# zhipeng-wei/Image-to-Video-I2V-attack

Hardware: AMD Instinct MI355X
Metric: adversarial frames/sec (10-step I2V, ResNet-50 layer3, 32x224^2 clips) (higher is better)
Workload: dtype f32

## Files before the change

image-to-video-i2v-attack_amd/csrc/i2v_conv_scpair.hip:

```cpp
#include "i2v_conv_tile.h"

#ifndef I2V_SCPAIR_WPE
#define I2V_SCPAIR_WPE I2V_PREF_WPE
#endif

template <int MODE_A>
__global__ void __launch_bounds__(256) __attribute__((amdgpu_waves_per_eu(I2V_SCPAIR_WPE, I2V_SCPAIR_WPE)))
conv_igemm_scpair(const I2VConvParams a, const I2VConvParams b, const int n_cd_tiles) {
    constexpr int BD = 64, BP = 64, WD = 2, WP = 2, FR = 32;
    constexpr bool PREF_A = MODE_A == 1;
    constexpr int LA = conv_lds_floats<BD, BP, WD, false, conv_deep(MODE_A, PREF_A) ? I2V_DEEP_STAGES : 2>();
    constexpr int LB = conv_lds_floats<BD, BP, WD, false, conv_deep(1, true) ? I2V_DEEP_STAGES : 2>();
    __shared__ __attribute__((aligned(16))) float smem[LA > LB ? LA : LB];
    I2V_PROBE_T probe;
    probe.entry();
    const int lid = conv_xcd_lid(blockIdx.x, gridDim.x);
    const int cd0 = (lid % n_cd_tiles) * BD;
    const int64_t px0 = (int64_t)(lid / n_cd_tiles) * BP;

    constexpr int C4 = BP / 4, RSTEP = 1024 / BP, NQ = WD * FR / RSTEP;
    float4 y[NQ];
    {
        f32x16 acc[1][1];
        float4 pre_a[PREF_A ? NQ : 1]; unsigned gw_a[PREF_A ? NQ : 1];
        conv_tile_loop<BD, BP, WD, WP, MODE_A, PREF_A>(a, cd0, px0, gridDim.x, smem, probe, blockIdx.x, I2V_PRIO_LEVELS, acc, pre_a, gw_a);
        float (*Cs)[BP] = reinterpret_cast<float (*)[BP]>(smem);
        conv_acc_to_rows<BP, WP, false>(acc[0], Cs);
        const int t = threadIdx.x, c4 = t % C4, rbase = t / C4;
        const bool pok = px0 + (int64_t)c4 * 4 < (int64_t)a.N * a.Hg * a.Wg;
#pragma unroll
        for (int q = 0; q < NQ; ++q) {
            const int row = rbase + q * RSTEP, cd = cd0 + row;
            float4 v = make_float4(0.f, 0.f, 0.f, 0.f);
            if (pok && cd < a.Cd) {
                v = *reinterpret_cast<const float4*>(&Cs[row][c4 * 4]);
                if (a.shift) { const float sh = a.shift[cd]; v.x += sh; v.y += sh; v.z += sh; v.w += sh; }
            }
            y[q] = v;
        }
        __syncthreads();
    }
    f32x16 acc[1][1];
    float4 pre0[NQ]; unsigned pregw[NQ];
    conv_tile_loop<BD, BP, WD, WP, 1, true>(b, cd0, px0, gridDim.x, smem, probe, blockIdx.x, I2V_PRIO_LEVELS, acc, pre0, pregw);
#pragma unroll
    for (int q = 0; q < NQ; ++q) pre0[q] = y[q];
    conv_vec_epilogue<BD, BP, WD, WP, true, false, false>(b, acc, cd0, px0, smem, pre0, pregw, nullptr);
    probe.exit(blockIdx.x);
}

long long g_stat_scpair = 0;

int k_conv_scpair_ok(const I2VConvParams& a, const I2VConvParams& b) { return i2v_conv_scpair_ok(a, b) ? 1 : 0; }

int k_conv_scpair(const I2VConvParams& a_in, const I2VConvParams& b_in, i2v_stream_t s) {
    I2VConvParams a = a_in, b = b_in;
    if (!i2v_conv_scpair_ok(a, b)) { snprintf(g_be_err, sizeof g_be_err, "shortcut-pair launch: the two launches do not form a pair"); g_be_has_err = true; return 1; }
    const int64_t P = (int64_t)b.N * b.Hg * b.Wg;
    if (P + 1024 >= (1ll << 31)) { snprintf(g_be_err, sizeof g_be_err, "conv launch of more than 2^31 grid pixels"); g_be_has_err = true; return 1; }
    conv_magics(a); conv_magics(b);
    b.add0 = nullptr; b.add0_nstride = 0;
    const int n_cd = (b.Cd + 63) / 64;
    const int64_t grid = (P + 63) / 64 * n_cd;
    if (grid <= 0) return 0;
    if (grid > 0x7fffffff) { snprintf(g_be_err, sizeof g_be_err, "conv grid too large"); g_be_has_err = true; return 1; }
    __atomic_fetch_add(&g_stat_scpair, 1, __ATOMIC_RELAXED);
    if (a.pointwise) hipLaunchKernelGGL((conv_igemm_scpair<1>), dim3((unsigned)grid), dim3(256), 0, (hipStream_t)s, a, b, n_cd);
    else hipLaunchKernelGGL((conv_igemm_scpair<2>), dim3((unsigned)grid), dim3(256), 0, (hipStream_t)s, a, b, n_cd);
    LAUNCH_CHECK("conv_scpair");
    return 0;
}
```

image-to-video-i2v-attack_amd/csrc/i2v_conv_tile.h:

```cpp
#pragma once
#include "i2v_be.h"

#ifndef I2V_PROBE_T
struct I2VNoProbe {
    __device__ __forceinline__ void entry() {}
    __device__ __forceinline__ void loop_begin() {}
    __device__ __forceinline__ void loop_end(int ) {}
    __device__ __forceinline__ void exit(int ) {}
};
#define I2V_PROBE_T I2VNoProbe
#endif

#ifndef I2V_PRIO_LEVELS
#define I2V_PRIO_LEVELS 3
#endif
#ifndef I2V_DEEP
#define I2V_DEEP 1
#endif
#ifndef I2V_DEEP_STAGES
#define I2V_DEEP_STAGES 3
#endif
#ifndef I2V_BF3_STAGES
#define I2V_BF3_STAGES 2
#endif
#ifndef I2V_SMALL_WPE
#define I2V_SMALL_WPE 7
#endif
#ifndef I2V_PREF_WPE
#define I2V_PREF_WPE 6
#endif
#ifndef I2V_MID_WPE
#define I2V_MID_WPE 5
#endif
#ifndef I2V_TALL_WPE
#define I2V_TALL_WPE 6
#endif
#ifndef I2V_BIG_WPE
#define I2V_BIG_WPE 3
#endif

static constexpr int conv_waves_per_simd(int BD, int BP, bool PREF, bool hi, int MODE = 0) {
    return (BD == 64 && BP == 64) ? (PREF ? (I2V_DEEP && MODE == 1 && I2V_DEEP_STAGES > 3 ? 4  : I2V_PREF_WPE) : I2V_SMALL_WPE) : (BD == 128 && BP == 64) ? I2V_TALL_WPE : (BD == 32 && BP == 256) ? 4  : BD * BP == 8192 ? I2V_MID_WPE : BD * BP == 16384 ? I2V_BIG_WPE : (hi ? 8 : 1);
}
#define I2V_CONV_WPE __attribute__((amdgpu_waves_per_eu(conv_waves_per_simd(BD, BP, PREF, false, MODE), conv_waves_per_simd(BD, BP, PREF, true, MODE))))
static constexpr bool conv_deep(int MODE, bool PREF) { return I2V_DEEP && PREF && MODE == 1; }
template <int BD, int BP, int WD, bool MF16, int NST = 2, int CPB = 1, int BF3 = 0>
constexpr int conv_lds_floats() {
    constexpr int stage = NST * CPB * (I2V_KC * BP + (BF3 == 2 ? 0 : BF3 ? ((BD / 32) * 3 + 3) / 4 * 4 * 256 : I2V_KC * BD)), epi = WD * (MF16 ? 16 : 32) * BP;
    return stage > epi ? stage : epi;
}

template <int HWM>
constexpr int conv_halo_lds_floats() {
    constexpr int stage = 2 * I2V_KC * (64 + 64 + 2 * HWM + 2), epi = 64 * 64;
    return stage > epi ? stage : epi;
}

template <int BD, int BP, int WD, bool PREF, bool MF16, bool FUSE, typename PT>
__device__ __forceinline__ void conv_vec_rows(const PT& p, const int i, const int cd0, const int64_t px0, const float (*const Cs)[BP], const int t,
                                              const float4* const pre0, const unsigned* const pregw, float* const mid) {
    constexpr int FR = MF16 ? 16 : 32;
    const int lane = t & 63;
    const int HWg = p.Hg * p.Wg, HoWo = p.Ho * p.Wo;
    const int64_t P = (int64_t)p.N * HWg;
    (void)pre0; (void)pregw; (void)mid;
#ifdef I2V_NT_ALL
    const bool nt_store = true;
#else
    const bool nt_store = p.cfg > 0 && ((p.cfg - 1) & 128);
#endif
    constexpr int C4 = BP / 4, RSTEP = 1024 / BP, NQ = WD * FR / RSTEP;
    const int c4 = t % C4, rbase = t / C4;
    const int64_t pp = px0 + (int64_t)c4 * 4;
    const bool pok = pp < P;
    const int64_t n = pok ? fastdiv((unsigned)pp, p.dv_hw_m, p.dv_hw_s) : 0;
    const int64_t poff = pp - n * HWg;
    #pragma unroll
    for (int q = 0; q < NQ; ++q) {
        const int row = rbase + q * RSTEP;
        const int cd = cd0 + (row / FR) * (BD / WD) + i * FR + (row % FR);
        const bool valid = pok && cd < p.Cd;
        float4 v = make_float4(0.f, 0.f, 0.f, 0.f);
        if (valid) {
        v = *reinterpret_cast<const float4*>(&Cs[row][c4 * 4]);
        const int64_t o = (int64_t)cd * HoWo + poff;
        if (p.gate_scale) {
            const float4 m = *reinterpret_cast<const float4*>(p.mask + n * p.mask_nstride + o);
            const float gs = p.gate_scale[cd], gt = p.gate_shift[cd];
            if (!(fmaf(m.x, gs, gt) > 0.f)) v.x = 0.f;
            if (!(fmaf(m.y, gs, gt) > 0.f)) v.y = 0.f;
            if (!(fmaf(m.z, gs, gt) > 0.f)) v.z = 0.f;
            if (!(fmaf(m.w, gs, gt) > 0.f)) v.w = 0.f;
        }
        if (p.shift) { const float sh = p.shift[cd]; v.x += sh; v.y += sh; v.z += sh; v.w += sh; }
        if (PREF) {
            v.x += pre0[q].x; v.y += pre0[q].y; v.z += pre0[q].z; v.w += pre0[q].w;
        } else {
            if (p.add0 && p.add0_stride == 1) {
                const float4 a = *reinterpret_cast<const float4*>(p.add0 + n * p.add0_nstride + o);
                v.x += a.x; v.y += a.y; v.z += a.z; v.w += a.w;
            } else if (p.add0) {
                const int oh = (int)fastdiv((unsigned)poff, p.dv_wo_m, p.dv_wo_s), ow = (int)(poff - (int64_t)oh * p.Wo);
                if (!(oh & 1) && (oh >> 1) < p.add0_H) {
                    const float2 a = *reinterpret_cast<const float2*>(
                        p.add0 + n * p.add0_nstride + (int64_t)cd * p.add0_H * p.add0_W + (oh >> 1) * p.add0_W + (ow >> 1));
                    v.x += a.x; v.z += a.y;
                }
            }
        }
        if (p.add1) {
            const float4 a = *reinterpret_cast<const float4*>(p.add1 + n * p.add1_nstride + o);
            v.x += a.x; v.y += a.y; v.z += a.z; v.w += a.w;
        }
        if (p.relu) { v.x = fmaxf(v.x, 0.f); v.y = fmaxf(v.y, 0.f); v.z = fmaxf(v.z, 0.f); v.w = fmaxf(v.w, 0.f); }
        if (p.gate) {
            const unsigned w = PREF ? pregw[q] : p.gate[(int64_t)cd * p.gate_stride + ((p.gate_pix0 + pp) >> 5)];
            const unsigned g = w >> ((unsigned)(p.gate_pix0 + pp) & 31u);
            if (!(g & 1u)) v.x = 0.f;
            if (!(g & 2u)) v.y = 0.f;
            if (!(g & 4u)) v.z = 0.f;
            if (!(g & 8u)) v.w = 0.f;
        } else if (p.mask && !p.gate_scale) {
            const float4 m = *reinterpret_cast<const float4*>(p.mask + n * p.mask_nstride + o);
            if (!(m.x > 0.f)) v.x = 0.f;
            if (!(m.y > 0.f)) v.y = 0.f;
            if (!(m.z > 0.f)) v.z = 0.f;
            if (!(m.w > 0.f)) v.w = 0.f;
        }
        if constexpr (!FUSE) {
            if (nt_store) { typedef float nt4 __attribute__((ext_vector_type(4))); const nt4 w4 = {v.x, v.y, v.z, v.w};
                            __builtin_nontemporal_store(w4, reinterpret_cast<nt4*>(p.dst + n * p.dst_nstride + o)); }
            else *reinterpret_cast<float4*>(p.dst + n * p.dst_nstride + o) = v;
        }
        }
        if constexpr (FUSE)
            *reinterpret_cast<float4*>(mid + (cd - cd0) * BP + c4 * 4) = v;
        if (p.gate_out) {
            unsigned nib = valid ? ((v.x > 0.f ? 1u : 0u) | (v.y > 0.f ? 2u : 0u) | (v.z > 0.f ? 4u : 0u) | (v.w > 0.f ? 8u : 0u)) : 0u;
            nib <<= 4 * (lane & 7);
            nib |= (unsigned)__builtin_amdgcn_update_dpp(0, (int)nib, 0xB1, 0xF, 0xF, true);
            nib |= (unsigned)__builtin_amdgcn_update_dpp(0, (int)nib, 0x4E, 0xF, 0xF, true);
            nib |= (unsigned)__builtin_amdgcn_update_dpp(0, (int)nib, 0x141, 0xF, 0xF, true);
            if (valid && (lane & 7) == 0)
                p.gate_out[(int64_t)cd * p.gate_out_stride + ((p.gate_out_pix0 + pp) >> 5)] = nib;
        }
    }
}

#define I2V_FROW(r) (MF16 ? 4 * lk + (r) : ((r) & 3) + 8 * ((r) >> 2) + 4 * lk)
template <int BP, int WP, bool MF16, int TP, typename ACC>
__device__ __forceinline__ void conv_acc_to_rows(ACC (&acc)[TP], float (*const Cs)[BP]) {
    constexpr int FR = MF16 ? 16 : 32, NR = MF16 ? 4 : 16;
    const int lane = threadIdx.x & 63, wave = threadIdx.x >> 6;
    const int wd = wave / WP, wpx = wave % WP;
    const int l31 = MF16 ? (lane & 15) : (lane & 31), lk = MF16 ? (lane >> 4) : (lane >> 5);
    __syncthreads();
#pragma unroll
    for (int j = 0; j < TP; ++j)
#pragma unroll
        for (int r = 0; r < NR; ++r)
            Cs[wd * FR + I2V_FROW(r)][wpx * (BP / WP) + j * FR + l31] = acc[j][r];
    __syncthreads();
}
template <int BD, int BP, int WD, int WP, bool PREF, bool MF16, bool FUSE, typename ACC, typename PT>
__device__ __forceinline__ void conv_vec_epilogue(const PT& p, ACC (&acc)[BD / WD / (MF16 ? 16 : 32)][BP / WP / (MF16 ? 16 : 32)], const int cd0,
                                                  const int64_t px0, float* const smem, const float4* const pre0, const unsigned* const pregw,
                                                  float* const mid) {
    constexpr int FR = MF16 ? 16 : 32, TD = BD / WD / FR;
    const int t = threadIdx.x;
    float (*Cs)[BP] = reinterpret_cast<float (*)[BP]>(smem);
#pragma unroll
    for (int i = 0; i < TD; ++i) {
        conv_acc_to_rows<BP, WP, MF16>(acc[i], Cs);
        conv_vec_rows<BD, BP, WD, PREF, MF16, FUSE>(p, i, cd0, px0, Cs, t, pre0, pregw, mid);
    }
}
#undef I2V_FROW

__device__ __forceinline__ int conv_xcd_lid(const int bid, const int nwg) {
    const int q8 = nwg >> 3, r8 = nwg & 7, xcd = bid & 7;
    return (xcd < r8 ? xcd * (q8 + 1) : r8 * (q8 + 1) + (xcd - r8) * q8) + (bid >> 3);
}

template <int BD, int BP, int WD, int WP, int MODE, bool PREF, bool PRE = false, bool VID = false, bool MF16 = false, int HWM = 0, int CPB = 1, int FUSE = 0, int BF3 = 0>
__device__ __forceinline__ void conv_tile_loop(const I2VConvParams& p, const int cd0, const int64_t px0, const int nwg, float* const smem, I2V_PROBE_T& probe,
                                               const int probe_slot, const int prio_arg,
                                               typename std::conditional<MF16, f32x4, f32x16>::type (&acc)[BD / WD / (MF16 ? 16 : 32)][BP / WP / (MF16 ? 16 : 32)],
                                               float4 (&pre0)[PREF ? WD * (MF16 ? 16 : 32) / (1024 / BP) : 1], unsigned (&pregw)[PREF ? WD * (MF16 ? 16 : 32) / (1024 / BP) : 1]) {
#if defined(__HIP_DEVICE_COMPILE__)
    constexpr int KC = I2V_KC;
    constexpr int FR = MF16 ? 16 : 32;
    constexpr int NR = MF16 ? 4 : 16;
    constexpr int TD = BD / WD / FR, TP = BP / WP / FR;
    static_assert(!(MF16 && (PRE || PREF)), "no pre-activation / prefetch variants of the 16x16 tile");
    constexpr bool DEEP = conv_deep(MODE, PREF) || (BF3 == 1 && I2V_BF3_STAGES > 2) || BF3 == 3;
    constexpr int NST = BF3 == 3 ? 3 : BF3 == 1 ? I2V_BF3_STAGES : DEEP ? I2V_DEEP_STAGES : 2, AHEAD = NST - 1;
    constexpr bool HALO = MODE == 5;
    constexpr int HS = HALO ? BP + 2 * HWM + 2 : 1, HQ = (HS + 63) / 64;
    static_assert(!HALO || (HWM > 0 && BD == 64 && BP == 64 && !PREF && !PRE && !VID && !MF16), "halo staging: the plain 64x64 image tile only");
    static_assert(CPB == 1 || (!HALO && !DEEP && !PREF && !PRE && MODE != 4 && MODE != 0), "several chunks per barrier: the plain pointwise / tap-uniform loops only");
    constexpr int KB = CPB * KC;
    static_assert(!BF3 || (!MF16 && !PRE && !PREF && !HALO && (MODE == 1 || MODE == 2) && FUSE == 0 && BD % 32 == 0), "split-bf16 K loop: the plain pointwise / tap-uniform tiles");
    constexpr int AF = BF3 == 2 ? 0 : BF3 ? CPB * (((BD / 32) * 3 + 3) / 4 * 4) * 256 : KB * BD;
    float (*As)[KB][BD] = reinterpret_cast<float (*)[KB][BD]>(smem);
    float* const As3 = smem;
    float (*Bs)[KB][BP] = reinterpret_cast<float (*)[KB][BP]>(smem + NST * AF);

    const int t = threadIdx.x, lane = t & 63, wave = t >> 6;
    const int wd = wave / WP, wpx = wave % WP;

    const int HWg = p.Hg * p.Wg;
    const int64_t P = (int64_t)p.N * HWg;

    constexpr bool PW = MODE == 1;
    constexpr bool QUAD = MODE == 4;
    typedef __attribute__((address_space(3))) void* lds_ptr_t;
    constexpr unsigned OOB = 0x80000000u;
    const int wv = __builtin_amdgcn_readfirstlane(wave);
    const __amdgpu_buffer_rsrc_t rs_w = BF3 ? __builtin_amdgcn_make_buffer_rsrc((void*)p.wp3, 0, (p.Kpad / KC) * (p.Cdpad / 32) * 3072, 0x00020000)
                                            : __builtin_amdgcn_make_buffer_rsrc((void*)p.wp, 0, p.Kpad * p.Cdpad * 4, 0x00020000);
    constexpr unsigned XB = QUAD ? 64u : 0u;
    const __amdgpu_buffer_rsrc_t rs_x = __builtin_amdgcn_make_buffer_rsrc((void*)((const char*)p.src - XB), 0, p.src_span_bytes + 2 * XB, 0x00020000);
    constexpr int NA = BF3 == 2 ? 0 : BF3 ? (BD / 32) * 3 : KC * BD / 256, NAQ = (NA + 3) / 4;
    constexpr int BPER = (PW || QUAD) ? 256 : 64;
    constexpr int NB = HALO ? 0 : KC * BP / BPER, NBQ = (NB + 3) / 4;
    const int bcol = PW ? (lane * 4) % BP : (BP >= 64 ? ((wave * 64) % BP) + lane : lane % BP);
    const int64_t ppix = px0 + bcol;
    const bool pvalid = ppix < P;
    const int64_t pn = pvalid ? fastdiv((unsigned)ppix, p.dv_hw_m, p.dv_hw_s) : 0;
    const int prem = (int)(ppix - pn * HWg);
    const int HWs = p.Hs * p.Ws;
    int h0 = 0, w0 = 0, t0 = 0;
    int64_t pns = pn;
    if (VID) {
        const int64_t clip = fastdiv((unsigned)pn, p.dv_t_m, p.dv_t_s);
        t0 = (int)(pn - clip * p.Tg) * p.st;
        pns = clip * p.Ts + t0;
    }
    const int nstr = (int)p.src_nstride;
    unsigned xoff;
    if (PW) xoff = (unsigned)((pns * p.src_nstride + prem) * 4);
    else {
        const int gi = (int)fastdiv((unsigned)prem, p.dv_w_m, p.dv_w_s), gj = prem - gi * p.Wg;
        h0 = gi * p.sh; w0 = gj * p.sw;
        xoff = (unsigned)((pns * p.src_nstride + (int64_t)h0 * p.Ws + w0) * 4) + XB;
    }
    if (!pvalid) xoff = OOB;
    unsigned aoff[NAQ ? NAQ : 1];
#pragma unroll
    for (int q = 0; q < NAQ; ++q) {
        const int f = (wave + 4 * q) * 256 + lane * 4;
        aoff[q] = BF3 ? (unsigned)(((cd0 / 32) * 3 + wave + 4 * q) * 1024 + lane * 16) : (unsigned)(((f / BD) * p.Cdpad + f % BD + cd0) * 4);
    }
    unsigned boff[PW ? NBQ : 1];
    if (PW) {
#pragma unroll
        for (int q = 0; q < NBQ; ++q) boff[q] = pvalid ? xoff + (unsigned)((((wave + 4 * q) * 256 + lane * 4) / BP) * HWs * 4) : OOB;
    }

#define I2V_ISSUE_PIECE(j_, k0_, buf_, vb_) I2V_ISSUE_PIECE_SUB(j_, k0_, buf_, vb_, 0)
#define I2V_ISSUE_PIECE_SUB(j_, k0_, buf_, vb_, sub_)                                                     \
    {                                                                                                     \
        constexpr int jj = (j_);                                                                          \
        const int k0 = (k0_);                                                                             \
        if constexpr (jj < NAQ) {                                                                         \
            const int ins = wv + 4 * jj;                                                                  \
            if constexpr (BF3) {    \
                __builtin_amdgcn_raw_ptr_buffer_load_lds(rs_w, (lds_ptr_t)(As3 + (buf_) * AF + (sub_) * (AF / CPB) + ins * 256), 16, ins < NA ? aoff[jj] : OOB, \
                                                         (k0 / KC) * (p.Cdpad / 32) * 3072, 0, 0);       \
            } else if (NA % 4 == 0 || ins < NA) {                                                         \
                if constexpr (false)                                                                      \
                    ;                                                                                     \
                else                                                                                      \
                    __builtin_amdgcn_raw_ptr_buffer_load_lds(rs_w, (lds_ptr_t)(&As[buf_][(sub_) * KC][0] + ins * 256), 16, aoff[jj],  \
                                                             k0 * p.Cdpad * 4, 0, 0);                     \
            }                                                                                             \
        } else {                                                                                          \
            constexpr int q = jj - NAQ;                                                                   \
            const int ins = wv + 4 * q;                                                                   \
            float* const bbuf = &Bs[buf_][(sub_) * KC][0];                                                \
            if (NB % 4 == 0 || ins < NB) {                                                                \
                if constexpr (PW) {                                                                       \
                    unsigned v = boff[q];                                                                 \
                    if (k0 + KC > p.K)             \
                        v = (k0 + ((wave + 4 * q) * 256 + lane * 4) / BP < p.K) ? v : OOB;                \
                    __builtin_amdgcn_raw_ptr_buffer_load_lds(rs_x, (lds_ptr_t)(bbuf + ins * 256), 16, v,         \
                                                             k0 * HWs * 4, 0, 0);                         \
                } else if constexpr (QUAD) {                                                              \
                     \
                    const I2VKEntry e = load_kentry(p.ktab, k0 + 4 * ((ins * 64) / BP));                  \
                    const int hs = h0 + e.dh, dtk = VID ? (e.valid >> 1) : 0;                             \
                    const bool ok = pvalid && (unsigned)hs < (unsigned)p.Hs && (!VID || (unsigned)(t0 + dtk) < (unsigned)p.Ts); \
                    const unsigned v = ok ? xoff + (unsigned)((e.chan_off + dtk * nstr + e.dh * p.Ws + e.dw) * 4) : OOB; \
                    __builtin_amdgcn_raw_ptr_buffer_load_lds(rs_x, (lds_ptr_t)(bbuf + ins * 256), 16, v, 0, 0, 0); \
                } else if constexpr (MODE == 2) {                                                         \
                    __builtin_amdgcn_raw_ptr_buffer_load_lds(rs_x, (lds_ptr_t)(bbuf + ins * 64), 4, vb_,         \
                                                             ((ins * 64) / BP) * HWs * 4, 0, 0);          \
                } else {                                                                                  \
                    const I2VKEntry e = load_kentry(p.ktab, k0 + (ins * 64) / BP);                        \
                    const int hs = h0 + e.dh, ws = w0 + e.dw, dtk = VID ? (e.valid >> 1) : 0;             \
                    const bool ok = pvalid && (e.valid & 1) && (unsigned)hs < (unsigned)p.Hs &&           \
                                    (unsigned)ws < (unsigned)p.Ws && (!VID || (unsigned)(t0 + dtk) < (unsigned)p.Ts); \
                    const unsigned v = ok ? xoff + (unsigned)((e.chan_off + dtk * nstr + e.dh * p.Ws + e.dw) * 4) : OOB; \
                    __builtin_amdgcn_raw_ptr_buffer_load_lds(rs_x, (lds_ptr_t)(bbuf + ins * 64), 4, v, 0, 0, 0); \
                }                                                                                         \
            }                                                                                             \
        }                                                                                                 \
    }
#define I2V_CHUNK_VB(e_)                                                                                  \
    ([&]() -> unsigned {                                                                                  \
        const int hs = h0 + (e_).dh, ws = w0 + (e_).dw, dtk = VID ? ((e_).valid >> 1) : 0;                \
        const bool ok = pvalid && (unsigned)hs < (unsigned)p.Hs && (unsigned)ws < (unsigned)p.Ws &&       \
                        (!VID || (unsigned)(t0 + dtk) < (unsigned)p.Ts);                                  \
        return ok ? xoff + (unsigned)(((e_).chan_off + dtk * nstr + (e_).dh * p.Ws + (e_).dw) * 4) : OOB; \
    }())

    constexpr int E_C4 = BP / 4, E_RSTEP = 1024 / BP, E_NQ = WD * FR / E_RSTEP;
    static_assert(!PREF || TD == 1, "PREF needs a single epilogue pass");
    static_assert(!PREF || E_NQ == WD * (MF16 ? 16 : 32) / (1024 / BP), "pre0 / pregw (the caller's): one entry per row a lane owns");
    if (PREF) {
        const int e_c4 = t % E_C4, e_rbase = t / E_C4;
        const int64_t e_pp = px0 + (int64_t)e_c4 * 4;
        const bool e_ok = e_pp < P;
        const int64_t e_n = e_ok ? fastdiv((unsigned)e_pp, p.dv_hw_m, p.dv_hw_s) : 0;
        const int64_t e_poff = e_pp - e_n * HWg;
        const int e_HoWo = p.Ho * p.Wo;
#pragma unroll
        for (int q = 0; q < E_NQ; ++q) {
            const int row = e_rbase + q * E_RSTEP;
            const int cd = cd0 + (row >> 5) * (BD / WD) + (row & 31);
            const bool ok = e_ok && cd < p.Cd;
            const int64_t o = (int64_t)cd * e_HoWo + e_poff;
            pre0[q] = (ok && p.add0) ? *reinterpret_cast<const float4*>(p.add0 + e_n * p.add0_nstride + o) : make_float4(0.f, 0.f, 0.f, 0.f);
            pregw[q] = (ok && p.gate) ? p.gate[(int64_t)cd * p.gate_stride + ((p.gate_pix0 + e_pp) >> 5)] : 0xffffffffu;
        }
    }

    probe.loop_begin();
    typedef short bf8 __attribute__((ext_vector_type(8)));
    typedef float f4 __attribute__((ext_vector_type(4)));
    constexpr int TD_ = BD / WD / (MF16 ? 16 : 32);
    bf8 wcur[BF3 == 2 ? CPB : 1][BF3 == 2 ? TD_ : 1][3];
    const char* const w3lane = BF3 ? (const char*)p.wp3 + (size_t)lane * 16 + (size_t)(cd0 / 32 + (wave / WP) * TD_) * 3072 : nullptr;
    const size_t w3chunk = BF3 ? (size_t)(p.Cdpad / 32) * 3072 : 0;
    auto load_w3 = [&](const int chunk, const int i, const int pl) {
        return __builtin_bit_cast(bf8, *reinterpret_cast<const f4*>(w3lane + (size_t)chunk * w3chunk + (i * 3 + pl) * 1024));
    };
    if constexpr (BF3 == 2) {
#pragma unroll
        for (int sb = 0; sb < CPB; ++sb)
#pragma unroll
            for (int i = 0; i < TD_; ++i)
#pragma unroll
                for (int pl = 0; pl < 3; ++pl) wcur[sb][i][pl] = load_w3(sb, i, pl);
    }
    (void)wcur; (void)w3lane; (void)w3chunk;
    constexpr int TP_ = BP / WP / (MF16 ? 16 : 32);
    bf8 xcur[BF3 == 3 ? TP_ : 1][3];
    (void)xcur;
    auto bf3_split2 = [](const float lo, const float hi, unsigned& p1, unsigned& p2, unsigned& p3) {
        typedef __bf16 bf2 __attribute__((ext_vector_type(2)));
        typedef float f2 __attribute__((ext_vector_type(2)));
        const unsigned a = __builtin_bit_cast(unsigned, __builtin_convertvector((f2){lo, hi}, bf2));
        const float rl = lo - __builtin_bit_cast(float, a << 16), rh = hi - __builtin_bit_cast(float, a & 0xffff0000u);
        const unsigned b = __builtin_bit_cast(unsigned, __builtin_convertvector((f2){rl, rh}, bf2));
        const float sl = rl - __builtin_bit_cast(float, b << 16), sh = rh - __builtin_bit_cast(float, b & 0xffff0000u);
        const unsigned c = __builtin_bit_cast(unsigned, __builtin_convertvector((f2){sl, sh}, bf2));
        p1 = a; p2 = b; p3 = c;
    };
    auto bf3_split_frag = [&](const float (&x)[8], bf8 (&out)[3]) {
        typedef unsigned u4 __attribute__((ext_vector_type(4)));
        unsigned q1[4], q2[4], q3[4];
#pragma unroll
        for (int e = 0; e < 4; ++e) bf3_split2(x[2 * e], x[2 * e + 1], q1[e], q2[e], q3[e]);
        out[0] = __builtin_bit_cast(bf8, (u4){q1[0], q1[1], q1[2], q1[3]});
        out[1] = __builtin_bit_cast(bf8, (u4){q2[0], q2[1], q2[2], q2[3]});
        out[2] = __builtin_bit_cast(bf8, (u4){q3[0], q3[1], q3[2], q3[3]});
    };
    (void)bf3_split_frag;
#pragma unroll
    for (int a = 0; a < TD; ++a)
#pragma unroll
        for (int b = 0; b < TP; ++b)
#pragma unroll
            for (int r = 0; r < NR; ++r) acc[a][b][r] = 0.f;

    const int nchunks = p.Kpad / KC;
    const int l31 = MF16 ? (lane & 15) : (lane & 31), lk = MF16 ? (lane >> 4) : (lane >> 5);
    constexpr int NL = NAQ + NBQ;
    constexpr int KR = MF16 ? 4 : 2;
    constexpr int KS = KC / KR;
    constexpr int PPS = (NL + KS - 1) / KS;
    I2VKEntry e_next[CPB];
#pragma unroll
    for (int h = 0; h < CPB; ++h) e_next[h] = I2VKEntry{0, 0, 0, 0};
    const int nsuper = nchunks / CPB;
    bool qok[QUAD ? TP : 1][2][MF16 ? 1 : 2];
    if constexpr (QUAD) {
#pragma unroll
        for (int j = 0; j < TP; ++j) {
            const int64_t fp = px0 + wpx * (BP / WP) + j * FR + l31;
            const unsigned fr = fp < P ? (unsigned)fp - fastdiv((unsigned)fp, p.dv_hw_m, p.dv_hw_s) * (unsigned)HWg : 0u;
            const int fj = (int)(fr - fastdiv(fr, p.dv_w_m, p.dv_w_s) * (unsigned)p.Wg);
#pragma unroll
            for (int qi = 0; qi < 2; ++qi)
#pragma unroll
                for (int hf = 0; hf < (MF16 ? 1 : 2); ++hf) {
                    const int el = MF16 ? lk : 2 * hf + lk;
                    qok[j][qi][hf] = 4 * qi + el < p.quad_kw && (unsigned)(fj * p.sw + p.quad_dw0 + 4 * qi + el) < (unsigned)p.Ws;
                }
        }
    }
    if constexpr (HALO) {
        constexpr int NT = 9, HPW = 4 * HQ, PPC = (HPW + NT - 1) / NT;
        float* const Hb = smem + NST * KC * BD;
        const int W_ = HWM;
        int tsh[NT], tdh[NT], tdw[NT];
#pragma unroll
        for (int t = 0; t < NT; ++t) {
            const I2VKEntry e = load_kentry(p.ktab, t * KC);
            tdh[t] = e.dh; tdw[t] = e.dw; tsh[t] = e.dh * W_ + e.dw + W_ + 1;
        }
        const int chan0 = load_kentry(p.ktab, 0).chan_off;
        const int ngroups = nchunks / NT;
        const int gstride = ngroups > 1 ? load_kentry(p.ktab, NT * KC).chan_off - chan0 : 0;
        const int64_t fp = px0 + wpx * (BP / WP) + l31;
        const bool fpv = fp < P;
        const unsigned fr = fpv ? (unsigned)fp - fastdiv((unsigned)fp, p.dv_hw_m, p.dv_hw_s) * (unsigned)HWg : 0u;
        const int fh = (int)fastdiv(fr, p.dv_w_m, p.dv_w_s), fw = (int)fr - fh * p.Wg;
        unsigned tmask = 0;
#pragma unroll
        for (int t = 0; t < NT; ++t)
            tmask |= (fpv && (unsigned)(fh + tdh[t]) < (unsigned)p.Hs && (unsigned)(fw + tdw[t]) < (unsigned)p.Ws) ? (1u << t) : 0u;
        const int lbase = lk * HS + wpx * (BP / WP) + l31;
        unsigned hoff[HQ];
#pragma unroll
        for (int q = 0; q < HQ; ++q) {
            const int64_t vp = px0 - (W_ + 1) + 64 * q + lane;
            const bool ok = vp >= 0 && vp < P;
            const int64_t vn = ok ? fastdiv((unsigned)vp, p.dv_hw_m, p.dv_hw_s) : 0;
            hoff[q] = ok ? (unsigned)((vn * p.src_nstride + (vp - vn * HWg)) * 4) : OOB;
        }
        auto halo_piece = [&]<int IDX>(std::integral_constant<int, IDX>, const int gb, const int chan_off) {
            constexpr int chl = IDX / HQ, q = IDX % HQ;
            float* const dst = Hb + ((gb * KC + wv * 4 + chl) * HS + 64 * q);
            const int so = (chan_off + (wv * 4 + chl) * HWs) * 4;
            if constexpr (chl == 3 && q == HQ - 1) {
                if (lane < HS - 64 * q) __builtin_amdgcn_raw_ptr_buffer_load_lds(rs_x, (lds_ptr_t)dst, 4, hoff[q], so, 0, 0);
            } else
                __builtin_amdgcn_raw_ptr_buffer_load_lds(rs_x, (lds_ptr_t)dst, 4, hoff[q], so, 0, 0);
        };
        if (ngroups > 0) {
            [&]<int... I>(std::integer_sequence<int, I...>) { ((halo_piece(std::integral_constant<int, I>{}, 0, chan0)), ...); }
            (std::make_integer_sequence<int, HPW>{});
            I2V_ISSUE_PIECE(0, 0, 0, OOB);
        }
        int gbuf = 0;
        for (int g = 0; g < ngroups; ++g) {
            const bool more_g = g + 1 < ngroups;
            const int chan_next = chan0 + (g + 1) * gstride;
            [&]<int... T>(std::integer_sequence<int, T...>) {
                (([&] {
                    constexpr int t = T;
                    const int abuf = (g + t) & 1;
                    asm volatile("s_waitcnt vmcnt(0)" ::: "memory");
                    asm volatile("s_waitcnt lgkmcnt(0)" ::: "memory");
                    __builtin_amdgcn_s_barrier();
                    const int hidx = lbase + gbuf * KC * HS + tsh[t];
                    const bool ok = (tmask >> t) & 1u;
                    float fa[2], fb[2];
                    auto rd = [&](const int s_, const int set) {
                        fa[set] = As[abuf][KR * s_ + lk][wd * (BD / WD) + l31];
                        fb[set] = Hb[hidx + KR * s_ * HS];
                    };
                    rd(0, 0);
                    [&]<int... S>(std::integer_sequence<int, S...>) {
                        (([&] {
                            constexpr int s_ = S, set = S & 1;
// ... 449 lines not shown
```

Measured before the change: 757.6.

## Split conv epilogue into load/math/store passes with early operand prefetch

Restructures the conv vector epilogue into separate operand-load, math and store phases, batched over row groups, so that global loads (shift, mask, residual, gate words) are issued before the accumulator-to-LDS barrier and overlap with it. The LDS staging barriers are replaced with explicit lgkmcnt waits plus raw s_barrier, which avoids waiting on outstanding global loads. The shortcut-pair kernel likewise prefetches shift values before the LDS transpose. The change adds register pressure from held operands and a configurable batching plan, while the 128x64 tile keeps the old chained path.

```diff
diff --git a/image-to-video-i2v-attack_amd/csrc/i2v_conv_scpair.hip b/image-to-video-i2v-attack_amd/csrc/i2v_conv_scpair.hip
--- a/image-to-video-i2v-attack_amd/csrc/i2v_conv_scpair.hip
+++ b/image-to-video-i2v-attack_amd/csrc/i2v_conv_scpair.hip
@@ -25,16 +25,21 @@
         float4 pre_a[PREF_A ? NQ : 1]; unsigned gw_a[PREF_A ? NQ : 1];
         conv_tile_loop<BD, BP, WD, WP, MODE_A, PREF_A>(a, cd0, px0, gridDim.x, smem, probe, blockIdx.x, I2V_PRIO_LEVELS, acc, pre_a, gw_a);
         float (*Cs)[BP] = reinterpret_cast<float (*)[BP]>(smem);
-        conv_acc_to_rows<BP, WP, false>(acc[0], Cs);
         const int t = threadIdx.x, c4 = t % C4, rbase = t / C4;
         const bool pok = px0 + (int64_t)c4 * 4 < (int64_t)a.N * a.Hg * a.Wg;
+        float sh[NQ];
+        if (a.shift) {
+#pragma unroll
+            for (int q = 0; q < NQ; ++q) { const int cd = cd0 + rbase + q * RSTEP; sh[q] = a.shift[cd < a.Cd ? cd : 0]; }
+        }
+        conv_acc_to_rows<BP, WP, false>(acc[0], Cs, t);
 #pragma unroll
         for (int q = 0; q < NQ; ++q) {
             const int row = rbase + q * RSTEP, cd = cd0 + row;
             float4 v = make_float4(0.f, 0.f, 0.f, 0.f);
             if (pok && cd < a.Cd) {
                 v = *reinterpret_cast<const float4*>(&Cs[row][c4 * 4]);
-                if (a.shift) { const float sh = a.shift[cd]; v.x += sh; v.y += sh; v.z += sh; v.w += sh; }
+                if (a.shift) { v.x += sh[q]; v.y += sh[q]; v.z += sh[q]; v.w += sh[q]; }
             }
             y[q] = v;
         }
diff --git a/image-to-video-i2v-attack_amd/csrc/i2v_conv_tile.h b/image-to-video-i2v-attack_amd/csrc/i2v_conv_tile.h
--- a/image-to-video-i2v-attack_amd/csrc/i2v_conv_tile.h
+++ b/image-to-video-i2v-attack_amd/csrc/i2v_conv_tile.h
@@ -56,8 +56,180 @@
     return stage > epi ? stage : epi;
 }
 
+struct ConvRowOps { float4 m, a0, a1; float gs, gt; unsigned gw; };
+template <int BP>
+struct ConvRowLane {
+    int c4, rbase;
+    int64_t pp, n, poff;
+    bool pok;
+    template <typename PT>
+    __device__ __forceinline__ ConvRowLane(const PT& p, const int64_t px0, const int t) {
+        c4 = t % (BP / 4); rbase = t / (BP / 4);
+        pp = px0 + (int64_t)c4 * 4;
+        pok = pp < (int64_t)p.N * (p.Hg * p.Wg);
+        n = pok ? fastdiv((unsigned)pp, p.dv_hw_m, p.dv_hw_s) : 0;
+        poff = pp - n * (p.Hg * p.Wg);
+    }
+};
+template <int BD, int BP, int WD, bool PREF, bool MF16, bool LITE, int NB, typename PT>
+__device__ __forceinline__ void conv_vec_rows_load(const PT& p, const int i, const int q0, const int cd0, const ConvRowLane<BP>& L, ConvRowOps (&ops)[NB],
+                                                   float (&sh)[WD * (MF16 ? 16 : 32) / (1024 / BP)]) {
+    constexpr int FR = MF16 ? 16 : 32, RSTEP = 1024 / BP, NQ = WD * FR / RSTEP;
+    const int HoWo = p.Ho * p.Wo;
+    int cdc[NB]; int64_t o[NB]; bool vld[NB];
+#pragma unroll
+    for (int q = 0; q < NB; ++q) {
+        const int row = L.rbase + (q0 + q) * RSTEP;
+        const int cd = cd0 + (row / FR) * (BD / WD) + i * FR + (row % FR);
+        const bool valid = L.pok && cd < p.Cd;
+        vld[q] = valid; cdc[q] = valid ? cd : 0;
+        o[q] = valid ? (int64_t)cd * HoWo + L.poff : 0;
+    }
+    if (!LITE && p.gate_scale) {
+#pragma unroll
+        for (int q = 0; q < NB; ++q) {
+            ops[q].m = *reinterpret_cast<const float4*>(p.mask + L.n * p.mask_nstride + o[q]);
+            ops[q].gs = p.gate_scale[(unsigned)cdc[q]]; ops[q].gt = p.gate_shift[(unsigned)cdc[q]];
+        }
+    }
+    if (LITE ? q0 == 0 && p.shift : p.shift != nullptr) {
+#pragma unroll
+        for (int q = LITE ? 0 : q0; q < (LITE ? NQ : q0 + NB); ++q) {
+            const int row = L.rbase + q * RSTEP;
+            const int cd = cd0 + (row / FR) * (BD / WD) + i * FR + (row % FR);
+            sh[q] = p.shift[cd < p.Cd ? (unsigned)cd : 0u];
+        }
+    }
+    if constexpr (!PREF) {
+        if (p.add0 && p.add0_stride == 1) {
+#pragma unroll
+            for (int q = 0; q < NB; ++q) ops[q].a0 = *reinterpret_cast<const float4*>(p.add0 + L.n * p.add0_nstride + o[q]);
+        } else if (p.add0) {
+            const int oh = (int)fastdiv((unsigned)L.poff, p.dv_wo_m, p.dv_wo_s), ow = (int)(L.poff - (int64_t)oh * p.Wo);
+            const bool even = !(oh & 1) && (oh >> 1) < p.add0_H;
+#pragma unroll
+            for (int q = 0; q < NB; ++q) {
+                const int64_t oc = (vld[q] && even)
+                                       ? L.n * p.add0_nstride + (int64_t)cdc[q] * p.add0_H * p.add0_W + (oh >> 1) * p.add0_W + (ow >> 1) : 0;
+                const float2 a = *reinterpret_cast<const float2*>(p.add0 + oc);
+                ops[q].a0.x = a.x; ops[q].a0.y = a.y;
+            }
+        }
+    }
+    if (p.add1) {
+#pragma unroll
+        for (int q = 0; q < NB; ++q) ops[q].a1 = *reinterpret_cast<const float4*>(p.add1 + L.n * p.add1_nstride + o[q]);
+    }
+    if (p.gate) {
+        if constexpr (!PREF) {
+            const int64_t gp = (int64_t)p.gate_pix0 + (L.pok ? L.pp : 0);
+#pragma unroll
+            for (int q = 0; q < NB; ++q) ops[q].gw = p.gate[(int64_t)cdc[q] * p.gate_stride + (gp >> 5)];
+        }
+    } else if (!LITE && p.mask && !p.gate_scale) {
+#pragma unroll
+        for (int q = 0; q < NB; ++q) ops[q].m = *reinterpret_cast<const float4*>(p.mask + L.n * p.mask_nstride + o[q]);
+    }
+}
+template <int BD, int BP, int WD, bool PREF, bool MF16, bool LITE, int NB, typename PT>
+__device__ __forceinline__ void conv_vec_rows_math(const PT& p, const int i, const int q0, const int cd0, const ConvRowLane<BP>& L, const float (*const Cs)[BP],
+                                                   const ConvRowOps (&ops)[NB], const float (&sh)[WD * (MF16 ? 16 : 32) / (1024 / BP)], const float4* const pre0,
+                                                   const unsigned* const pregw, float4 (&vv)[NB]) {
+    constexpr int FR = MF16 ? 16 : 32, RSTEP = 1024 / BP;
+    (void)pre0; (void)pregw;
+#pragma unroll
+    for (int q = 0; q < NB; ++q) {
+        const int row = L.rbase + (q0 + q) * RSTEP;
+        const int cd = cd0 + (row / FR) * (BD / WD) + i * FR + (row % FR);
+        const bool valid = L.pok && cd < p.Cd;
+        float4 v = make_float4(0.f, 0.f, 0.f, 0.f);
+        if (valid) {
+        v = *reinterpret_cast<const float4*>(&Cs[row][L.c4 * 4]);
+        if (!LITE && p.gate_scale) {
+            const float4 m = ops[q].m;
+            const float gs = ops[q].gs, gt = ops[q].gt;
+            if (!(fmaf(m.x, gs, gt) > 0.f)) v.x = 0.f;
+            if (!(fmaf(m.y, gs, gt) > 0.f)) v.y = 0.f;
+            if (!(fmaf(m.z, gs, gt) > 0.f)) v.z = 0.f;
+            if (!(fmaf(m.w, gs, gt) > 0.f)) v.w = 0.f;
+        }
+        if (p.shift) { const float s = sh[q0 + q]; v.x += s; v.y += s; v.z += s; v.w += s; }
+        if (PREF) {
+            v.x += pre0[q0 + q].x; v.y += pre0[q0 + q].y; v.z += pre0[q0 + q].z; v.w += pre0[q0 + q].w;
+        } else {
+            if (p.add0 && p.add0_stride == 1) {
+                const float4 a = ops[q].a0;
+                v.x += a.x; v.y += a.y; v.z += a.z; v.w += a.w;
+            } else if (p.add0) {
+                const int oh = (int)fastdiv((unsigned)L.poff, p.dv_wo_m, p.dv_wo_s);
+                if (!(oh & 1) && (oh >> 1) < p.add0_H) { v.x += ops[q].a0.x; v.z += ops[q].a0.y; }
+            }
+        }
+        if (p.add1) {
+            const float4 a = ops[q].a1;
+            v.x += a.x; v.y += a.y; v.z += a.z; v.w += a.w;
+        }
+        if (p.relu) { v.x = fmaxf(v.x, 0.f); v.y = fmaxf(v.y, 0.f); v.z = fmaxf(v.z, 0.f); v.w = fmaxf(v.w, 0.f); }
+        if (p.gate) {
+            const unsigned w = PREF ? pregw[q0 + q] : ops[q].gw;
+            const unsigned g = w >> (((unsigned)p.gate_pix0 + (unsigned)L.pp) & 31u);
+            if (!(g & 1u)) v.x = 0.f;
+            if (!(g & 2u)) v.y = 0.f;
+            if (!(g & 4u)) v.z = 0.f;
+            if (!(g & 8u)) v.w = 0.f;
+        } else if (!LITE && p.mask && !p.gate_scale) {
+            const float4 m = ops[q].m;
+            if (!(m.x > 0.f)) v.x = 0.f;
+            if (!(m.y > 0.f)) v.y = 0.f;
+            if (!(m.z > 0.f)) v.z = 0.f;
+            if (!(m.w > 0.f)) v.w = 0.f;
+        }
+        }
+        vv[q] = v;
+    }
+}
+template <int BD, int BP, int WD, bool MF16, bool FUSE, int NB, typename PT>
+__device__ __forceinline__ void conv_vec_rows_store(const PT& p, const int i, const int q0, const int cd0, const ConvRowLane<BP>& L, const float4 (&vv)[NB],
+                                                    const int t, float* const mid) {
+    constexpr int FR = MF16 ? 16 : 32, RSTEP = 1024 / BP;
+    const int lane = t & 63;
+    const int HoWo = p.Ho * p.Wo;
+    (void)mid;
+#ifdef I2V_NT_ALL
+    const bool nt_store = true;
+#else
+    const bool nt_store = p.cfg > 0 && ((p.cfg - 1) & 128);
+#endif
+#pragma unroll
+    for (int q = 0; q < NB; ++q) {
+        const int row = L.rbase + (q0 + q) * RSTEP;
+        const int cd = cd0 + (row / FR) * (BD / WD) + i * FR + (row % FR);
+        const bool valid = L.pok && cd < p.Cd;
+        const float4 v = vv[q];
+        if constexpr (!FUSE) {
+            if (valid) {
+            const int64_t o = (int64_t)cd * HoWo + L.poff;
+            if (nt_store) { typedef float nt4 __attribute__((ext_vector_type(4))); const nt4 w4 = {v.x, v.y, v.z, v.w};
+                            __builtin_nontemporal_store(w4, reinterpret_cast<nt4*>(p.dst + L.n * p.dst_nstride + o)); }
+            else *reinterpret_cast<float4*>(p.dst + L.n * p.dst_nstride + o) = v;
+            }
+        }
+        if constexpr (FUSE)
+            *reinterpret_cast<float4*>(mid + (cd - cd0) * BP + L.c4 * 4) = v;
+        if (p.gate_out) {
+            unsigned nib = valid ? ((v.x > 0.f ? 1u : 0u) | (v.y > 0.f ? 2u : 0u) | (v.z > 0.f ? 4u : 0u) | (v.w > 0.f ? 8u : 0u)) : 0u;
+            nib <<= 4 * (lane & 7);
+            nib |= (unsigned)__builtin_amdgcn_update_dpp(0, (int)nib, 0xB1, 0xF, 0xF, true);
+            nib |= (unsigned)__builtin_amdgcn_update_dpp(0, (int)nib, 0x4E, 0xF, 0xF, true);
+            nib |= (unsigned)__builtin_amdgcn_update_dpp(0, (int)nib, 0x141, 0xF, 0xF, true);
+            if (valid && (lane & 7) == 0)
+                p.gate_out[(int64_t)cd * p.gate_out_stride + (((int64_t)p.gate_out_pix0 + L.pp) >> 5)] = nib;
+        }
+    }
+}
+
 template <int BD, int BP, int WD, bool PREF, bool MF16, bool FUSE, typename PT>
-__device__ __forceinline__ void conv_vec_rows(const PT& p, const int i, const int cd0, const int64_t px0, const float (*const Cs)[BP], const int t,
+__device__ __forceinline__ void conv_vec_rows_chain(const PT& p, const int i, const int cd0, const int64_t px0, const float (*const Cs)[BP], const int t,
                                               const float4* const pre0, const unsigned* const pregw, float* const mid) {
     constexpr int FR = MF16 ? 16 : 32;
     const int lane = t & 63;
@@ -149,31 +321,79 @@
 
 #define I2V_FROW(r) (MF16 ? 4 * lk + (r) : ((r) & 3) + 8 * ((r) >> 2) + 4 * lk)
 template <int BP, int WP, bool MF16, int TP, typename ACC>
-__device__ __forceinline__ void conv_acc_to_rows(ACC (&acc)[TP], float (*const Cs)[BP]) {
+__device__ __forceinline__ void conv_acc_to_rows(ACC (&acc)[TP], float (*const Cs)[BP], const int t) {
     constexpr int FR = MF16 ? 16 : 32, NR = MF16 ? 4 : 16;
-    const int lane = threadIdx.x & 63, wave = threadIdx.x >> 6;
+    const int lane = t & 63, wave = t >> 6;
     const int wd = wave / WP, wpx = wave % WP;
     const int l31 = MF16 ? (lane & 15) : (lane & 31), lk = MF16 ? (lane >> 4) : (lane >> 5);
-    __syncthreads();
+    asm volatile("s_waitcnt lgkmcnt(0)" ::: "memory");
+    __builtin_amdgcn_s_barrier();
+    asm volatile("" ::: "memory");
 #pragma unroll
     for (int j = 0; j < TP; ++j)
 #pragma unroll
         for (int r = 0; r < NR; ++r)
             Cs[wd * FR + I2V_FROW(r)][wpx * (BP / WP) + j * FR + l31] = acc[j][r];
-    __syncthreads();
+    asm volatile("s_waitcnt lgkmcnt(0)" ::: "memory");
+    __builtin_amdgcn_s_barrier();
+    asm volatile("" ::: "memory");
+}
+struct ConvEpiPlan { int nb; bool ahead, early; };
+#ifndef I2V_EPI_PLAN
+template <int BD, int BP, bool LITE>
+constexpr ConvEpiPlan conv_epi_plan() {
+    if (BD == 128 && BP == 128) return {2, true, true};
+    if (!LITE) return {1, false, true};
+    return {2, false, true};
+}
+#else
+template <int BD, int BP, bool LITE>
+constexpr ConvEpiPlan conv_epi_plan() { return I2V_EPI_PLAN; }
+#endif
+template <int BD, int BP, int WD, int WP, bool PREF, bool MF16, bool FUSE, bool LITE, typename ACC, typename PT>
+__device__ __forceinline__ void conv_vec_passes(const PT& p, ACC (&acc)[BD / WD / (MF16 ? 16 : 32)][BP / WP / (MF16 ? 16 : 32)], const int cd0,
+                                                const int64_t px0, float (*const Cs)[BP], const int t, const float4* const pre0,
+                                                const unsigned* const pregw, float* const mid) {
+    constexpr int FR = MF16 ? 16 : 32, TD = BD / WD / FR, NQ = WD * FR / (1024 / BP);
+    constexpr ConvEpiPlan PL = conv_epi_plan<BD, BP, LITE>();
+    constexpr int NB = NQ < PL.nb ? NQ : PL.nb, NBP = NQ / NB, NBT = TD * NBP;
+    static_assert(NQ % NB == 0, "a pass is a whole number of row batches");
+    const ConvRowLane<BP> L(p, px0, t);
+    ConvRowOps ops[NB];
+    float sh[NQ];
+    float4 v[NB];
+    if constexpr (PL.early) conv_vec_rows_load<BD, BP, WD, PREF, MF16, LITE>(p, 0, 0, cd0, L, ops, sh);
+#pragma unroll
+    for (int b = 0; b < NBT; ++b) {
+        const int i = b / NBP, q0 = (b % NBP) * NB;
+        if (q0 == 0) {
+            conv_acc_to_rows<BP, WP, MF16>(acc[i], Cs, t);
+            if constexpr (!PL.early) conv_vec_rows_load<BD, BP, WD, PREF, MF16, LITE>(p, i, 0, cd0, L, ops, sh);
+        }
+        conv_vec_rows_math<BD, BP, WD, PREF, MF16, LITE>(p, i, q0, cd0, L, Cs, ops, sh, pre0, pregw, v);
+        const bool next = b + 1 < NBT && (PL.early || (b + 1) % NBP != 0);
+        if (PL.ahead && next) conv_vec_rows_load<BD, BP, WD, PREF, MF16, LITE>(p, (b + 1) / NBP, ((b + 1) % NBP) * NB, cd0, L, ops, sh);
+        conv_vec_rows_store<BD, BP, WD, MF16, FUSE>(p, i, q0, cd0, L, v, t, mid);
+        if (!PL.ahead && next) conv_vec_rows_load<BD, BP, WD, PREF, MF16, LITE>(p, (b + 1) / NBP, ((b + 1) % NBP) * NB, cd0, L, ops, sh);
+    }
 }
 template <int BD, int BP, int WD, int WP, bool PREF, bool MF16, bool FUSE, typename ACC, typename PT>
 __device__ __forceinline__ void conv_vec_epilogue(const PT& p, ACC (&acc)[BD / WD / (MF16 ? 16 : 32)][BP / WP / (MF16 ? 16 : 32)], const int cd0,
                                                   const int64_t px0, float* const smem, const float4* const pre0, const unsigned* const pregw,
                                                   float* const mid) {
-    constexpr int FR = MF16 ? 16 : 32, TD = BD / WD / FR;
+    float (*Cs)[BP] = reinterpret_cast<float (*)[BP]>(smem);
     const int t = threadIdx.x;
-    float (*Cs)[BP] = reinterpret_cast<float (*)[BP]>(smem);
-#pragma unroll
-    for (int i = 0; i < TD; ++i) {
-        conv_acc_to_rows<BP, WP, MF16>(acc[i], Cs);
-        conv_vec_rows<BD, BP, WD, PREF, MF16, FUSE>(p, i, cd0, px0, Cs, t, pre0, pregw, mid);
-    }
+    if constexpr (BD == 128 && BP == 64) {
+        constexpr int TD = BD / WD / (MF16 ? 16 : 32);
+#pragma unroll
+        for (int i = 0; i < TD; ++i) {
+            conv_acc_to_rows<BP, WP, MF16>(acc[i], Cs, t);
+            conv_vec_rows_chain<BD, BP, WD, PREF, MF16, FUSE>(p, i, cd0, px0, Cs, t, pre0, pregw, mid);
+        }
+        return;
+    }
+    if (p.gate_scale || (p.mask && !p.gate)) conv_vec_passes<BD, BP, WD, WP, PREF, MF16, FUSE, false>(p, acc, cd0, px0, Cs, t, pre0, pregw, mid);
+    else conv_vec_passes<BD, BP, WD, WP, PREF, MF16, FUSE, true>(p, acc, cd0, px0, Cs, t, pre0, pregw, mid);
 }
 #undef I2V_FROW
 
```

Measured after the change: 749.3. -1.1%, worse.
